# GuoleiSun/VSS-CFFM

Measured on AMD Instinct MI355X. Metric: clips/sec (fwd+bwd) CFFM-B1 480x480 T=4 hot path (CFFA+CFM, decoder_focal depth 2), higher is better.
Workload: dtype f32 in/out, f32 accumulate; MFMA operands: split-bf16 (hi+lo, ~2^-17) in the Linear GEMMs, f16 in QK^T/AV

## Files before the change

vss_cffm_amd/csrc/cffm_hip.hip:

```cpp
#include "cfm_attn_kernels.h"
#include "clip_kernels.h"
#include "rowops_kernels.h"
#include "gtc_kernels.h"
#include "gemm.h"
#include "segfuse_kernels.h"
#include "segloss_kernels.h"
#include "headfuse_kernels.h"

#include <stdarg.h>
#include <stdio.h>

#include "../../include/cffm_hip.h"

static thread_local char g_err[512] = "";

static int fail(int code, const char* fmt, ...) {
    va_list ap;
    va_start(ap, fmt);
    vsnprintf(g_err, sizeof(g_err), fmt, ap);
    va_end(ap);
    return code;
}
#define CHECK_LAUNCH(name)                                                                        \
    do {                                                                                          \
// ... 873 lines not shown
    ScratchFor pool(stream);
    PROF(ST_GEMM);
    if (gemm_tn_group((const GemmTN*)problems, n, (hipStream_t)stream)) return fail(-3, "linear_bwd_weight_group: gemm failed");
    CHECK_LAUNCH("linear_bwd_weight_group");
    return 0;
}

long cffm_tfrag_floats(long R, int C) { return R < 0 || C < 16 ? 0 : ((R + 31) / 32) * 32 * (long)C; }
int cffm_tfrag_pack(const float* x, float* dst, long R, int C, void* stream) {
    REQUIRE(x && dst && R >= 1 && C >= 16 && C % 16 == 0, "tfrag_pack: C must be a multiple of 16");
    const long items = ((R + 31) / 32) * (C / 16) * 64;
    CFFM_LAUNCH(k_tfrag_pack, ((unsigned)((items + 255) / 256)), (256), 0, (hipStream_t)stream, x, R, C, 0, (f32x4*)dst, items);
    CHECK_LAUNCH("tfrag_pack");
    return 0;
}
int cffm_linear_bwd_weight_tfrag_group(const cffm_wgrad* problems, int n, void* stream) {
    REQUIRE(problems && n >= 1 && n <= DWS_MAX, "linear_bwd_weight_tfrag_group: 1..%d problems", DWS_MAX);
    for (int i = 0; i < n; ++i) REQUIRE(problems[i].dy && problems[i].x && problems[i].dw, "linear_bwd_weight_tfrag_group: null operand");
    PROF(ST_GEMM);
    DwsPlan P;
    REQUIRE(dw_stream_plan((const GemmTN*)problems, n, dw_stream_target(), &P), "linear_bwd_weight_tfrag_group: N must be a multiple of 64, K of 128, operands under 4 GB");
    float* part = P.part_floats ? lib_scratch(P.part_floats) : nullptr;
    REQUIRE(!P.part_floats || part, "linear_bwd_weight_tfrag_group: scratch allocation failed");
    REQUIRE(!dw_group_stream((const GemmTN*)problems, n, (hipStream_t)stream, part, dw_stream_target()), "linear_bwd_weight_tfrag_group: launch failed");
    CHECK_LAUNCH("linear_bwd_weight_tfrag_group");
    return 0;
}
int cffm_linear_bwd_weight_tfrag(const float* dy_t, const float* x_t, float* dw, long M, int N, int K, void* stream) {
    const cffm_wgrad pr = {dy_t, x_t, dw, M, N, K};
    return cffm_linear_bwd_weight_tfrag_group(&pr, 1, stream);
}

int cffm_linear_qkv_fwd(const float* x, const float* w, const float* b, void* qkv16, long M, void* stream) {
    REQUIRE(x && w && b && qkv16, "linear_qkv_fwd: null");
    PROF(ST_GEMM);
    return gemm_nt_qkv16_split(x, w, b, (h16*)qkv16, M, 768, CFFM_C, (hipStream_t)stream) ? fail(-3, "linear_qkv_fwd: gemm failed") : 0;
}

int cffm_colsum(const float* a, long rows, int cols, float* out, void* stream) {
    ScratchFor pool(stream);
    PROF(ST_COLSUM);
    hipStream_t st = (hipStream_t)stream;
    REQUIRE(a && out && cols >= 4 && cols % 4 == 0, "colsum: cols must be a multiple of 4");
    const int slices = (int)((rows + COLSUM_ROWS - 1) / COLSUM_ROWS);
    float* part = red_scratch((size_t)slices * cols, st);
    REQUIRE(part, "colsum: scratch allocation failed");
    CFFM_LAUNCH(k_colsum_partial, (slices), (256), 0, st, a, rows, cols, part);
    RedSegs segs;
    segs.nseg = 0;
    seg_add(segs, 0, cols, out, 0);
    reduce_records(part, slices, cols, cols, segs, st);
    CHECK_LAUNCH("colsum");
    return 0;
}

static int cffm_ln_bwd_residual(const float* x1, const float* mean, const float* rstd, const float* gamma, const float* dz2,
                                const float* dres, float* dx1, float* dgamma, float* dbeta, long nrows, int zero_grads,
                                float* dres_colsum, float* dx1_colsum, void* stream) {
    PROF(ST_LN_BWD);
    hipStream_t st = (hipStream_t)stream;
    const int rpb = LNB_ROWS;
    const int nblk = (int)((nrows + rpb - 1) / rpb);
    float* part = red_scratch((size_t)nblk * 1024, st);
    REQUIRE(part, "ln_bwd_residual: scratch allocation failed");
    CFFM_LAUNCH(k_ln_bwd_residual, (nblk), (256), 0, st, x1, mean, rstd, gamma, dz2, dres, dx1, part, nrows, rpb);
    RedSegs segs;
    segs.nseg = 0;
    seg_add(segs, 0, CFFM_C, dgamma, !zero_grads);
    seg_add(segs, CFFM_C, CFFM_C, dbeta, !zero_grads);
    seg_add(segs, 2 * CFFM_C, CFFM_C, dres_colsum, 0);
    seg_add(segs, 3 * CFFM_C, CFFM_C, dx1_colsum, 0);
    reduce_records(part, nblk, 1024, 1024, segs, st);
    CHECK_LAUNCH("ln_bwd_residual");
    return 0;
}


int cffm_adamw_step_rows(const cffm_adamw_chunk2* chunks, int nchunks, const float* grad_base, float* state, const float* sched,
                         double* consts, int nrows, const int* active_rows, int* ticket, void* stream) {
    static_assert(sizeof(cffm_adamw_chunk2) == sizeof(AdamwChunk2), "chunk layout");
    if (nchunks <= 0) return 0;
    REQUIRE(chunks && state && sched && consts && nrows >= 1, "adamw_step_rows: null table or no rows");
    PROF(ST_ADAMW);
    if (ticket) {
        CFFM_LAUNCH(k_adamw_rows_tick, ((unsigned)nchunks), (256), 0, (hipStream_t)stream, (const AdamwChunk2*)chunks, grad_base, state, sched, consts,
                    nrows, active_rows, ticket);
    } else {
        CFFM_LAUNCH(k_adamw_tick_rows, ((unsigned)((nrows + 63) / 64)), (64), 0, (hipStream_t)stream, state, sched, consts, nrows, active_rows);
        CFFM_LAUNCH(k_adamw_rows, ((unsigned)nchunks), (256), 0, (hipStream_t)stream, (const AdamwChunk2*)chunks, grad_base, (const float*)state, consts);
    }
    CHECK_LAUNCH("adamw_rows");
    return 0;
}

#ifndef GTM_WGS_FWD
#define GTM_WGS_FWD 512
#endif
#ifndef GTM_WGS_DQ
#define GTM_WGS_DQ 512
#endif
#ifndef GTM_WGS_DKV
#define GTM_WGS_DKV 256
#endif
int cffm_gtc_attn_fwd(const float* q_raw, const float* q_b, const float* kv_raw, const float* kv_b, float* o, float* lse,
                      int B, int T, int K, void* stream) {
    PROF(ST_GTC_FWD);
    REQUIRE(K >= 1 && K <= 256, "gtc_attn_fwd: K=%d outside 1..256", K);
#ifndef CFFM_EMU
    static bool granted = false;
    if (!granted) {
        REQUIRE(hipFuncSetAttribute((const void*)k_gtc_attn_fwd, hipFuncAttributeMaxDynamicSharedMemorySize, gtf_lds(256)) == hipSuccess, "gtc_attn_fwd: LDS grant failed");
        granted = true;
    }
#endif
    if (K <= 128) {
        const int tiles = (T + 15) / 16;
        int tpw = (tiles * CFFM_HEADS * B + 4 * GTM_WGS_FWD - 1) / (4 * GTM_WGS_FWD);
        if (tpw < 1) tpw = 1;
        const unsigned gx = (unsigned)((tiles + 4 * tpw - 1) / (4 * tpw));
        const int U = (K + 31) / 32;
        hipStream_t st = (hipStream_t)stream;
        f32x4* fr = (f32x4*)lib_scratch((size_t)B * CFFM_HEADS * gtm_frag_units(U) * 256);
        REQUIRE(fr, "gtc_attn_fwd: scratch allocation failed");
#define GTM_FWD(U_)                                                                                                                          \
        do {                                                                                                                             \
            if (U_ > 1) CFFM_LAUNCH(k_gtc_pack_frags<U_>, (CFFM_HEADS, B, 2 * U_), (256), 0, st, kv_raw, kv_b, fr, K);                   \
            CFFM_LAUNCH(k_gtc_attn_fwd_mfma<U_>, (gx, CFFM_HEADS, B), (256), 0, st, q_raw, q_b, (const f32x4*)(U_ > 1 ? fr : nullptr), kv_raw, kv_b, o, lse, T, K, tpw);   \
        } while (0)
        if (U == 1) GTM_FWD(1); else if (U == 2) GTM_FWD(2); else if (U == 3) GTM_FWD(3); else GTM_FWD(4);
#undef GTM_FWD
        CHECK_LAUNCH("gtc_attn_fwd");
        return 0;
    }
    CFFM_LAUNCH(k_gtc_attn_fwd, ((T + GTC_TOK - 1) / GTC_TOK, CFFM_HEADS, B), (256), (size_t)gtf_lds(K), (hipStream_t)stream, q_raw, q_b, kv_raw, kv_b, o,
                lse, T, K);
    CHECK_LAUNCH("gtc_attn_fwd");
    return 0;
}

int cffm_gtc_attn_bwd(const float* q_raw, const float* q_b, const float* kv_raw, const float* kv_b, const float* o,
                      const float* dout, const float* lse, float* dq_raw, float* dkv, int B, int T, int K, void* stream) {
    PROF(ST_GTC_BWD);
    hipStream_t st = (hipStream_t)stream;
    REQUIRE(K >= 1 && K <= 256 && B >= 1 && T >= 1, "gtc_attn_bwd: K=%d outside 1..256", K);
    if (K <= 128) {
        const int tiles = (T + 15) / 16, pairs = (T + 31) / 32, U = (K + 31) / 32;
        int tpw = (tiles * CFFM_HEADS * B + 4 * GTM_WGS_DQ - 1) / (4 * GTM_WGS_DQ), ppw = (pairs * CFFM_HEADS * B + 4 * GTM_WGS_DKV - 1) / (4 * GTM_WGS_DKV);
        if (tpw < 1) tpw = 1;
        if (ppw < 1) ppw = 1;
        const unsigned g1 = (unsigned)((tiles + 4 * tpw - 1) / (4 * tpw)), g2 = (unsigned)((pairs + 4 * ppw - 1) / (4 * ppw));
        const size_t nD = ((size_t)B * T * CFFM_HEADS + 63) / 64 * 64;
        const size_t nrecf = ((size_t)B * CFFM_HEADS * g2 * K * 64 + 63) / 64 * 64;
        float* scr = lib_scratch(nD + nrecf + (size_t)B * CFFM_HEADS * gtm_frag_units(U) * 256);
        REQUIRE(scr, "gtc_attn_bwd: scratch allocation failed");
        float* Dbuf = scr;
        float* rec = scr + nD;
        f32x4* fr = (f32x4*)(scr + nD + nrecf);
#ifndef CFFM_EMU
        static bool granted_m = false;
        if (!granted_m) {
            REQUIRE(hipFuncSetAttribute((const void*)k_gtc_attn_bwd_dkv_mfma<3>, hipFuncAttributeMaxDynamicSharedMemorySize, gtm_bwd_lds(4)) == hipSuccess &&
                    hipFuncSetAttribute((const void*)k_gtc_attn_bwd_dkv_mfma<4>, hipFuncAttributeMaxDynamicSharedMemorySize, gtm_bwd_lds(4)) == hipSuccess, "gtc_attn_bwd: LDS grant failed");
            granted_m = true;
        }
#endif
#define GTM_BWD(U_)                                                                                                                                              \
        do {                                                                                                                                                 \
            const f32x4* fq = U_ > 1 ? (const f32x4*)fr : nullptr;                                \
            if (U_ > 1) CFFM_LAUNCH(k_gtc_pack_frags<U_>, (CFFM_HEADS, B, 2 * U_), (256), 0, st, kv_raw, kv_b, fr, K);                                       \
// ... 223 lines not shown
    }
    TRY(cffm_gtc_attn_fwd(ws + W.qraw, p->qkv_b, ws + W.kvraw, p->kv_b, ws + W.ao, ws + W.lse, B, T, K, stream));
    TRY(cffm_mlp_fwd_tfrag(ws + W.ao, x, 0, (int)nt, wf + 256 * 256, wf + 2 * 256 * 256, wf + 2 * 256 * 256 + CFFM_HID * 256, p->proj_b, p->fc1_b, p->fc2_b,
                           p->norm2_w, p->norm2_b, ws + W.x1, nullptr, ws + W.mean2, ws + W.rstd2, ws + W.hraw, nullptr, out, ws + W.ao_t, ws + W.z2,
                           ws + W.act, nt, stream));
    return 0;
}

int cffm_gtc_block_backward(const cffm_gtc_params* p, const cffm_gtc_grads* g, const float* x, const float* centers, const float* dout,
                            float* dx, float* dcenters, float* ws, int B, int T, int K, void* stream) {
    TRY(gtc_check(p, x, centers, dout, ws, B, T, K, "gtc_block_backward"));
    REQUIRE(g && dx && dcenters && g->norm1_w && g->norm1_b && g->qkv_w && g->qkv_b && g->kv_w && g->kv_b && g->proj_w && g->proj_b && g->norm2_w &&
            g->norm2_b && g->fc1_w && g->fc1_b && g->fc2_w && g->fc2_b, "gtc_block_backward: null gradient");
    hipStream_t st = (hipStream_t)stream;
    const long nt = (long)B * T, nk = (long)B * K;
    const GtcWs W = gtc_ws_layout(nt, nk);
    float* wn = ws + W.wn;
    TRY(gtc_pack(p, wn, 1, stream));
#ifdef CFFM_EMU
    memset(g->qkv_w + 256 * 256, 0, sizeof(float) * 512 * 256);
    memset(g->qkv_b + 256, 0, sizeof(float) * 512);
#else
    REQUIRE(hipMemsetAsync(g->qkv_w + 256 * 256, 0, sizeof(float) * 512 * 256, st) == hipSuccess &&
            hipMemsetAsync(g->qkv_b + 256, 0, sizeof(float) * 512, st) == hipSuccess, "gtc_block_backward: memset failed");
#endif
    RedScope reductions(st);
    TRY(cffm_mlp_bwd_tfrag(dout, ws + W.hraw, p->fc1_b, ws + W.x1, ws + W.mean2, ws + W.rstd2, p->norm2_w, wn + 2 * 256 * 256 + CFFM_HID * 256,
                           wn + 2 * 256 * 256, wn + 256 * 256, nullptr, ws + W.dx1, ws + W.dao, g->norm2_w, g->norm2_b, g->fc1_b, g->fc2_b, g->proj_b,
                           ws + W.dout_t, ws + W.dh, ws + W.dx1_t, nt, stream));
    TRY(cffm_gtc_attn_bwd(ws + W.qraw, p->qkv_b, ws + W.kvraw, p->kv_b, ws + W.ao, ws + W.dao, ws + W.lse, ws + W.dq, ws + W.dkv, B, T, K, stream));
    {
        PROF(ST_GEMM);
        const int mt = panel_mt(nt);
        const long nrec = (nt + 16 * mt - 1) / (16 * mt);
        float* qrec = red_scratch((size_t)nrec * 256, st);
        REQUIRE(qrec, "gtc_block_backward: scratch allocation failed");
        float* dq_t = ws + W.dq_t;
        const int rc = mt == 3 ? panel_gemm_launch<3, 2, false, 0>(ws + W.dq, 256, nt, 256, wn, ws + W.dz, 256, nullptr, nullptr, st, qrec, dq_t)
                               : panel_gemm_launch<2, 2, false, 0>(ws + W.dq, 256, nt, 256, wn, ws + W.dz, 256, nullptr, nullptr, st, qrec, dq_t);
        REQUIRE(!rc, "gtc_block_backward: q input-gradient gemm failed");
        RedSegs segs;
        segs.nseg = 0;
        seg_add(segs, 0, 256, g->qkv_b, 0);
        reduce_records(qrec, (int)nrec, 256, 256, segs, st);
    }
    {
        PROF(ST_GEMM); PROF2(ST_G_DW);
        const cffm_wgrad wt4[4] = {{ws + W.dq_t, ws + W.z_t, g->qkv_w, nt, 256, 256}, {ws + W.dh, ws + W.z2, g->fc1_w, nt, CFFM_HID, 256},
                                   {ws + W.dout_t, ws + W.act, g->fc2_w, nt, 256, CFFM_HID}, {ws + W.dx1_t, ws + W.ao_t, g->proj_w, nt, 256, 256}};
        DwsPlan P;
        REQUIRE(dw_stream_plan((const GemmTN*)wt4, 4, dw_stream_target(), &P), "gtc_block_backward: weight-gradient plan failed");
        float* part = P.part_floats ? lib_scratch(P.part_floats) : nullptr;
        REQUIRE(!P.part_floats || part, "gtc_block_backward: scratch allocation failed");
        REQUIRE(!dw_group_stream((const GemmTN*)wt4, 4, st, part, dw_stream_target()), "gtc_block_backward: weight-gradient gemm failed");
    }
    TRY(cffm_colsum(ws + W.dkv, nk, 512, g->kv_b, stream));
    {
        PROF(ST_GEMM);
        REQUIRE(!gemm_tn(ws + W.dkv, ws + W.cn, g->kv_w, nk, 512, 256, st), "gtc_block_backward: kv weight-gradient gemm failed");
        REQUIRE(!gemm_nn(ws + W.dkv, p->kv_w, ws + W.dcn, nk, 512, 256, st), "gtc_block_backward: kv input-gradient gemm failed");
    }
    TRY(cffm_ln_bwd_residual(x, ws + W.mean1, ws + W.rstd1, p->norm1_w, ws + W.dz, ws + W.dx1, dx, g->norm1_w, g->norm1_b, nt, 1, nullptr, nullptr, stream));
    reductions.finish();
    TRY(cffm_ln_bwd_residual(centers, ws + W.cmean, ws + W.crstd, p->norm1_w, ws + W.dcn, nullptr, dcenters, g->norm1_w, g->norm1_b, nk, 0, nullptr, nullptr,
                             stream));
    CHECK_LAUNCH("gtc_block_backward");
    return 0;
}

static int prep_args(PrepArgs& a, const cffm_block_params* params, int d0, int nd, float* ws0, long ws_stride, const cffm_block_ws& L) {
    const int nb = (CFFM_HEADS * CFFM_NQ_PAD * CFFM_NKEY_PAD + 255) / 256;
    for (int d = 0; d < PREP_MAXD; ++d) {
        const cffm_block_params& p = params[d0 + (d < nd ? d : 0)];
        float* ws = ws0 + (long)(d0 + (d < nd ? d : 0)) * ws_stride;
        a.t[d].own = p.rpb_own; a.t[d].ring = p.rpb_ring;
        for (int i = 0; i < 4; ++i) { a.t[d].pool[i] = p.rpb_pool[i]; a.pw[d].w[i] = p.pool_w[i]; }
        a.bias[d] = ws + L.bias; a.M[d] = ws + L.M;
        a.w[d][0] = p.qkv_w; a.w[d][1] = p.proj_w; a.w[d][2] = p.fc1_w; a.w[d][3] = p.fc2_w;
        a.w_s[d] = ws + L.w_split;
        a.w_f[d] = ws + L.w_frag;
    }
    a.nbias = nb;
    a.pack = 2;
    return nb + 1 + PREP_WBLOCKS + PREP_FBLOCKS;
}
static int param_prep(const cffm_block_params* params, int n, float* ws0, long ws_stride, const cffm_block_ws& L, void* stream) {
    PROF(ST_BIAS_ASM);
    for (int d0 = 0; d0 < n; d0 += PREP_MAXD) {
        const int nd = (n - d0 < PREP_MAXD) ? n - d0 : PREP_MAXD;
        PrepArgs a;
        const int pnx = prep_args(a, params, d0, nd, ws0, ws_stride, L);
        CFFM_LAUNCH(k_param_prep, (pnx, nd), (256), 0, (hipStream_t)stream, a);
    }
    CHECK_LAUNCH("param_prep");
    return 0;
}

static int block_forward_impl(const cffm_geom* g, const cffm_block_params* p, const float* x_ref, long ref_bs,
                              const float* x_tgt, long tgt_bs, const int* key_src, const int* q_dst, float* ws,
                              float* scratch, void* stream);
int cffm_block_forward(const cffm_geom* g, const cffm_block_params* p, const float* x_ref, long ref_bs,
                       const float* x_tgt, long tgt_bs, const int* key_src, const int* q_dst, float* ws,
                       float* scratch, void* stream) {
    REQUIRE(g && p && ws && scratch, "block_forward: null");
    cffm_block_ws L;
    cffm_block_ws_layout(g, &L);
    TRY(param_prep(p, 1, ws, 0, L, stream));
    return block_forward_impl(g, p, x_ref, ref_bs, x_tgt, tgt_bs, key_src, q_dst, ws, scratch, stream);
}
static struct { bool pending; hipStream_t side; } g_prep_join = {false, nullptr};
static int block_forward_impl(const cffm_geom* g, const cffm_block_params* p, const float* x_ref, long ref_bs,
                              const float* x_tgt, long tgt_bs, const int* key_src, const int* q_dst, float* ws,
                              float* scratch, void* stream) {
    cffm_block_ws L;
    cffm_block_ws_layout(g, &L);
    const long NR = (long)g->B * g->RC, NP = (long)g->B * g->HW;
    hipStream_t st = (hipStream_t)stream;
    const bool late_join = g_prep_join.pending;
    TRY(ln_pool_fwd_impl(g, x_ref, ref_bs, x_tgt, tgt_bs, p->norm1_w, p->norm1_b, ws + L.M, p->pool_b, ws + L.zall,
                         ws + L.mean1, ws + L.rstd1, 1, stream, late_join ? p->pool_w : nullptr));
    if (late_join) {
        g_prep_join.pending = false;
        side_join(g_prep_join.side, st, 0);
    }
    {
        PROF(ST_GEMM); PROF2(ST_G_QKV_FWD);
        REQUIRE(!panel_qkv_fwd(ws + L.zall, ws + L.w_frag, p->qkv_b, (h16*)(ws + L.qkv), NR, st, dw_stream_sw() ? ws + L.zall_t : nullptr), "block_forward: qkv gemm failed");
    }
    TRY(cffm_attn_fwd(g, ws + L.qkv, key_src, q_dst, (const void*)(ws + L.bias), ws + L.ao, ws + L.lse, stream));
    {
        const float* wf = ws + L.w_frag;
        PROF(ST_GEMM);
        if (dw_stream_sw())
            TRY(cffm_mlp_fwd_tfrag(ws + L.ao, x_tgt, tgt_bs, g->HW, wf + 768 * 256, wf + 768 * 256 + 256 * 256, wf + 768 * 256 + 256 * 256 + 1024 * 256,
                                   p->proj_b, p->fc1_b, p->fc2_b, p->norm2_w, p->norm2_b, ws + L.x1, nullptr, ws + L.mean2, ws + L.rstd2, ws + L.hraw,
                                   nullptr, ws + L.x2, ws + L.ao_t, ws + L.z2, ws + L.act, NP, stream));
        else
        TRY(cffm_mlp_fwd(ws + L.ao, x_tgt, tgt_bs, g->HW, wf + 768 * 256, wf + 768 * 256 + 256 * 256, wf + 768 * 256 + 256 * 256 + 1024 * 256,
                         p->proj_b, p->fc1_b, p->fc2_b, p->norm2_w, p->norm2_b, ws + L.x1, ws + L.z2, ws + L.mean2, ws + L.rstd2, ws + L.hraw,
                         ws + L.act, ws + L.x2, NP, stream));
        CHECK_LAUNCH("block_forward");
    }
    (void)scratch;
    return 0;
}

static int block_backward_impl(const cffm_geom* g, const cffm_block_params* p, const cffm_block_grads* gr,
                               const float* x_ref, long ref_bs, const float* x_tgt, long tgt_bs, const int* key_src,
                               const int* q_dst, const int* inv_ptr, const int* inv_idx, const float* ws, const float* dout,
                               float* dx_tgt, long dtgt_bs, float* scratch, int defer, int par, int slot, int nslots, void* stream);
#ifndef CFFM_EMU
static struct { bool has; RedJobs jobs; int parity; } g_tail = {false, {}, 0};
static int tail_flush(hipStream_t st) {
    if (!g_tail.has) return 0;
    g_tail.has = false;
    hipStream_t s3 = side_fork_take(st, 3);
    (void)hipStreamWaitEvent(s3, g_side.tail_order, 0);
    redq_launch(g_tail.jobs, s3);
    CHECK_LAUNCH("block_backward reductions");
    if (s3 != st) {
        side_record(s3, st, g_side.tail_done[g_tail.parity]);
        g_side.tail_pending[g_tail.parity] = true;
    }
    return 0;
}
#else
static int tail_flush(hipStream_t) { return 0; }
// ... 613 lines not shown
int cffm_vc_counts(const long long* gt, const long long* pred, int F, long npix, int n, long long* counts, void* stream) {
    REQUIRE(F >= 0 && npix >= 0 && n >= 1 && npix < (1L << 31), "vc_counts: bad sizes");
    if (F - n <= 0 || !npix) return 0;
    REQUIRE(gt && pred && counts, "vc_counts: null");
    REQUIRE(F - n <= 65535, "vc_counts: more than 65535 start frames in one call");
    CFFM_LAUNCH(k_vc_counts, ((unsigned)((npix + 255) / 256), (unsigned)(F - n)), (256), 0, (hipStream_t)stream, gt, pred, npix, n,
                (unsigned long long*)counts);
    CHECK_LAUNCH("vc_counts");
    return 0;
}

int cffm_layer_forward_rows(const cffm_geom* g, int depth, const cffm_block_params* params, const float* x_rows, float* y_rows,
                            const int* key_src, const int* q_dst, float* saved, float* scratch, void* stream) {
    REQUIRE(g && params && x_rows && y_rows && saved && scratch && depth >= 1, "layer_forward_rows: bad arguments");
    cffm_block_ws L;
    cffm_block_ws_layout(g, &L);
    const long HW = g->HW, img = HW * CFFM_C;
    float* blk0 = saved + up((long)g->B * 4 * img);
    TRY(param_prep(params, depth, blk0, L.total, L, stream));
    for (int i = 0; i < depth; ++i) {
        float* ws = blk0 + (long)i * L.total;
        const float* tgt = (i == 0) ? x_rows + 3 * img : blk0 + (long)(i - 1) * L.total + L.x2;
        const long tgt_bs = (i == 0) ? 4 * img : img;
        TRY(block_forward_impl(g, &params[i], x_rows, 4 * img, tgt, tgt_bs, key_src, q_dst, ws, scratch, stream));
    }
#ifdef CFFM_EMU
    memcpy(y_rows, blk0 + (long)(depth - 1) * L.total + L.x2, (size_t)g->B * img * sizeof(float));
#else
    REQUIRE(hipMemcpyAsync(y_rows, blk0 + (long)(depth - 1) * L.total + L.x2, (size_t)g->B * img * sizeof(float), hipMemcpyDeviceToDevice,
                           (hipStream_t)stream) == hipSuccess, "layer_forward_rows: copy failed");
#endif
    return 0;
}
int cffm_layer_backward_rows(const cffm_geom* g, int depth, const cffm_block_params* params, const cffm_block_grads* grads,
                             const float* x_rows, const float* dy_rows, float* dx_rows, const int* key_src, const int* q_dst,
                             const int* inv_ptr, const int* inv_idx, const float* saved, float* scratch, void* stream) {
    REQUIRE(g && params && grads && x_rows && dy_rows && dx_rows && saved && scratch && depth >= 1, "layer_backward_rows: bad arguments");
    cffm_block_ws L;
    cffm_block_ws_layout(g, &L);
    const Scratch S = scratch_layout(g);
    const long HW = g->HW, img = HW * CFFM_C;
    const float* blk0 = saved + up((long)g->B * 4 * img);
    tail_reset();
    for (int i = depth - 1; i >= 0; --i) {
        const float* ws = blk0 + (long)i * L.total;
        const float* tgt = (i == 0) ? x_rows + 3 * img : blk0 + (long)(i - 1) * L.total + L.x2;
        const long tgt_bs = (i == 0) ? 4 * img : img;
        float* dtgt = (i == 0) ? dx_rows + 3 * img : scratch + (((depth - i) & 1) ? S.a2 : S.a);
        const long dtgt_bs = (i == 0) ? 4 * img : img;
        const float* dout = (i == depth - 1) ? dy_rows : scratch + (((depth - 1 - i) & 1) ? S.a2 : S.a);
        TRY(block_backward_impl(g, &params[i], &grads[i], x_rows, 4 * img, tgt, tgt_bs, key_src, q_dst, inv_ptr, inv_idx, ws, dout, dtgt, dtgt_bs,
                                scratch, 1, (depth - 1 - i) & 1, i, depth, stream));
    }
    RedJobs* tail_jobs = nullptr;
#ifndef CFFM_EMU
    if (g_tail.has) {
        g_tail.has = false;
        tail_jobs = &g_tail.jobs;
    }
#endif
    TRY(cffa_finish(g, depth, params, grads, depth - 1, 0, blk0, L.total, x_rows, 4 * img, dx_rows, 4 * img, 0, stream, tail_jobs));
    side_join_all((hipStream_t)stream);
    return 0;
}

static int layer_forward_impl(const cffm_geom* g, int depth, const cffm_block_params* params, const float* x_nchw,
                              float* y_tgt_nchw, long y_bs, float* y_full, const int* key_src, const int* q_dst, float* saved,
                              float* scratch, void* stream) {
    REQUIRE(g && params && x_nchw && y_tgt_nchw && saved && scratch && depth >= 1, "layer_forward: bad arguments");
    cffm_block_ws L;
    cffm_block_ws_layout(g, &L);
    const long HW = g->HW, img = HW * CFFM_C;
    float* xs = saved;
    float* blk0 = saved + up((long)g->B * 4 * img);
    hipStream_t st = (hipStream_t)stream;
    side_init(st);
    if (depth <= PREP_MAXD) {
        PROF(ST_TRANSPOSE);
        PrepArgs a;
        const int pnx = prep_args(a, params, 0, depth, blk0, L.total, L);
        TrArgs T;
        T.src = x_nchw; T.dst = xs; T.rows = CFFM_C; T.cols = (int)HW; T.src_bs = img; T.dst_bs = img; T.add_mod = 4; T.add_skip = 3; T.copy_dst = y_full;
        T.gx = ((int)HW + 63) / 64; T.gy = (CFFM_C + 63) / 64; T.gz = g->B * 4;
        CFFM_LAUNCH(k_transpose_prep, ((unsigned)(T.gx * T.gy * T.gz + pnx * depth)), (256), 0, st, T, a, pnx);
        CHECK_LAUNCH("transpose + param_prep");
        g_prep_join.pending = false;
    } else {
        side_fork_mark(st, 0);
        TRY(transpose_add(x_nchw, xs, g->B * 4, CFFM_C, (int)HW, img, img, nullptr, 4, 3, stream, y_full));
        hipStream_t sd = side_fork_take(st, 0);
        TRY(param_prep(params, depth, blk0, L.total, L, (void*)sd));
        side_mark(sd, st, 0);
        g_prep_join.pending = sd != st;
        g_prep_join.side = sd;
    }
#ifndef CFFM_EMU
    g_side.used = 0;
#endif
    for (int i = 0; i < depth; ++i) {
        float* ws = blk0 + (long)i * L.total;
        const float* tgt = (i == 0) ? xs + 3 * img : blk0 + (long)(i - 1) * L.total + L.x2;
        const long tgt_bs = (i == 0) ? 4 * img : img;
        TRY(block_forward_impl(g, &params[i], xs, 4 * img, tgt, tgt_bs, key_src, q_dst, ws, scratch, stream));
    }
    TRY(cffm_transpose(blk0 + (long)(depth - 1) * L.total + L.x2, y_tgt_nchw, g->B, (int)HW, CFFM_C, img, y_bs, stream));
    return 0;
}
int cffm_layer_forward(const cffm_geom* g, int depth, const cffm_block_params* params, const float* x_nchw,
                       float* y_tgt_nchw, const int* key_src, const int* q_dst, float* saved, float* scratch,
                       void* stream) {
    REQUIRE(g, "layer_forward: bad arguments");
    return layer_forward_impl(g, depth, params, x_nchw, y_tgt_nchw, g->HW * CFFM_C, nullptr, key_src, q_dst, saved, scratch, stream);
}
int cffm_layer_forward_full(const cffm_geom* g, int depth, const cffm_block_params* params, const float* x_nchw,
                            float* y_full_nchw, const int* key_src, const int* q_dst, float* saved, float* scratch,
                            void* stream) {
    REQUIRE(g && y_full_nchw && y_full_nchw != x_nchw, "layer_forward_full: bad arguments");
    const long img = g->HW * CFFM_C;
    return layer_forward_impl(g, depth, params, x_nchw, y_full_nchw + 3 * img, 4 * img, y_full_nchw, key_src, q_dst, saved, scratch, stream);
}

static int layer_backward_impl(const cffm_geom* g, int depth, const cffm_block_params* params, const cffm_block_grads* grads,
                               const float* dy_tgt_nchw, long dy_bs, const float* dy_full, float* dx_nchw, const int* key_src,
                               const int* q_dst, const int* inv_ptr, const int* inv_idx, const float* saved, float* scratch,
                               int first_block, int last_block, void* stream) {
    REQUIRE(g && params && grads && dy_tgt_nchw && dx_nchw && saved && scratch && depth >= 1, "layer_backward: bad arguments");
    REQUIRE(first_block < depth && last_block >= 0 && first_block >= last_block, "layer_backward: bad block range %d..%d of %d", first_block,
            last_block, depth);
    cffm_block_ws L;
    cffm_block_ws_layout(g, &L);
    const Scratch S = scratch_layout(g);
    const long HW = g->HW, img = HW * CFFM_C;
    const float* xs = saved;
    const float* blk0 = saved + up((long)g->B * 4 * img);
    float* dxs = scratch + S.dxs;
    REQUIRE(dy_bs >= img, "layer_backward: dy batch stride %ld < %ld", dy_bs, img);
    if (first_block == depth - 1) TRY(cffm_transpose(dy_tgt_nchw, scratch + S.a, g->B, CFFM_C, (int)HW, dy_bs, img, stream));
    tail_reset();
    for (int i = first_block; i >= last_block; --i) {
        const float* ws = blk0 + (long)i * L.total;
        const float* tgt = (i == 0) ? xs + 3 * img : blk0 + (long)(i - 1) * L.total + L.x2;
        const long tgt_bs = (i == 0) ? 4 * img : img;
        float* dcur = scratch + (((depth - 1 - i) & 1) ? S.a2 : S.a);
        float* dtgt = (i == 0) ? dxs + 3 * img : scratch + (((depth - i) & 1) ? S.a2 : S.a);
        const long dtgt_bs = (i == 0) ? 4 * img : img;
        TRY(block_backward_impl(g, &params[i], &grads[i], xs, 4 * img, tgt, tgt_bs, key_src, q_dst, inv_ptr, inv_idx, ws, dcur, dtgt, dtgt_bs, scratch,
                                1, (depth - 1 - i) & 1, i, depth, stream));
    }
    RedJobs* tail_jobs = nullptr;
#ifndef CFFM_EMU
    if (last_block == 0 && g_tail.has) {
        g_tail.has = false;
        tail_jobs = &g_tail.jobs;
    }
#endif
    TRY(cffa_finish(g, depth, params, grads, first_block, last_block, blk0, L.total, xs, 4 * img, dxs, 4 * img, first_block != depth - 1, stream, tail_jobs));
    if (last_block == 0) TRY(transpose_add(dxs, dx_nchw, g->B * 4, (int)HW, CFFM_C, img, img, dy_full, 4, 3, stream));
    TRY(tail_flush((hipStream_t)stream));
    side_join_all((hipStream_t)stream);
    return 0;
}
int cffm_layer_backward_range(const cffm_geom* g, int depth, const cffm_block_params* params, const cffm_block_grads* grads,
                              const float* dy_tgt_nchw, long dy_bs, float* dx_nchw, const int* key_src, const int* q_dst,
                              const int* inv_ptr, const int* inv_idx, const float* saved, float* scratch, int first_block,
                              int last_block, void* stream) {
    return layer_backward_impl(g, depth, params, grads, dy_tgt_nchw, dy_bs, nullptr, dx_nchw, key_src, q_dst, inv_ptr, inv_idx, saved,
                               scratch, first_block, last_block, stream);
// ... 22 lines not shown
```

vss_cffm_amd/csrc/rowops_kernels.h:

```cpp
#pragma once
#include "cffm_common.h"
#include "cffa_kernels.h"
#include "panel_kernels.h"

struct BiasTables {
    const float* own;
    const float* ring;
    const float* pool[4];
};
struct BiasTablesG {
    float* own;
    float* ring;
    float* pool[4];
};

__device__ __forceinline__ int bias_locate(int h, int q, int n, int& off) {
    const int qi = q / 7, qj = q % 7;
    if (n < 49) {
        const int ki = n / 7, kj = n % 7;
        off = ((qi - ki + 6) * 13 + (qj - kj + 6)) * CFFM_HEADS + h;
        return 0;
    }
    if (n < 181) {
        off = (h * 49 + q) * 132 + (n - 49);
        return 1;
    }
    int base, kk, id;
    if (n < 206) { base = 181; kk = 5; id = 2; }
    else if (n < 255) { base = 206; kk = 7; id = 3; }
    else if (n < 280) { base = 255; kk = 5; id = 4; }
    else { base = 280; kk = 3; id = 5; }
    const int a = (n - base) / kk, bb = (n - base) % kk, side = 6 + kk;
    off = h * side * side + (qi - a + kk - 1) * side + (qj - bb + kk - 1);
    return id;
}

__device__ __forceinline__ long biash_index(int h, int q, int n) {
    const int t = n >> 4;
    return ((long)((h * 4 + (q >> 4)) * 10 + (t >> 1)) * 64 + (((t & 1) * 2 + ((n >> 3) & 1)) * 16 + (q & 15))) * 8 + (n & 7);
}
__device__ __forceinline__ void bias_assemble_body(const BiasTables& t, float* __restrict__ bias, h16* __restrict__ biasH, int bx) {
    const int e = bx * 256 + threadIdx.x;
    if (e >= CFFM_HEADS * CFFM_NQ_PAD * CFFM_NKEY_PAD) return;
    const int n = e % CFFM_NKEY_PAD, q = (e / CFFM_NKEY_PAD) % CFFM_NQ_PAD, h = e / (CFFM_NKEY_PAD * CFFM_NQ_PAD);
    float v = 0.f;
    if (q < CFFM_WA && n < CFFM_NKEY) {
        int off;
        const int id = bias_locate(h, q, n, off);
        v = id == 0 ? t.own[off] : id == 1 ? t.ring[off] : t.pool[id - 2][off];
    }
    if (bias) bias[e] = v;
    if (biasH) {
        biasH[biash_index(h, q, n)] = (h16)v;
        if (n >= CFFM_NKEY_PAD - 16) biasH[biash_index(h, q, n + 16)] = (h16)0.f;
    }
}
__global__ void __launch_bounds__(256) k_bias_assemble(BiasTables t, float* __restrict__ bias, h16* __restrict__ biasH) {
    bias_assemble_body(t, bias, biasH, blockIdx.x);
}
#define PREP_MAXD 4
#define PREP_WFLOATS (768 * 256 + 256 * 256 + 1024 * 256 + 256 * 1024)
#define PREP_WBLOCKS (PREP_WFLOATS / 4 / 256)
#define PREP_FBLOCKS (2 * PREP_WFLOATS / 8 / 256)
struct PrepArgs {
    BiasTables t[PREP_MAXD];
    PoolW pw[PREP_MAXD];
    float* bias[PREP_MAXD];
    float* M[PREP_MAXD];
    const float* w[PREP_MAXD][4];
    float* w_s[PREP_MAXD];
    float* w_f[PREP_MAXD];
    int nbias, pack;
};
__device__ __forceinline__ void param_prep_body(const PrepArgs& a, int bx, int d) {
    if (bx < a.nbias) { bias_assemble_body(a.t[d], nullptr, (h16*)a.bias[d], bx); return; }
    if (bx == a.nbias) { pool_matrix_body(a.pw[d], a.M[d]); return; }
    if (!a.pack) return;
    const long n4[4] = {768 * 256 / 4, 256 * 256 / 4, 1024 * 256 / 4, 256 * 1024 / 4};
    if (bx >= a.nbias + 1 + PREP_WBLOCKS) {
        long it = (long)(bx - a.nbias - 1 - PREP_WBLOCKS) * 256 + threadIdx.x;
        const int form = it >= PREP_WFLOATS / 8;
        if (form) it -= PREP_WFLOATS / 8;
        const int N[4] = {768, 256, 1024, 256}, K[4] = {256, 256, 256, 1024};
        long o8 = 0;
#pragma unroll
        for (int k = 0; k < 4; ++k) {
            if (it >= o8 && it < o8 + n4[k] / 2)
                pnl_pack_weight(a.w[d][k], N[k], K[k], form != 0, (f32x4*)(a.w_f[d] + (long)form * PREP_WFLOATS + o8 * 8), it - o8);
            o8 += n4[k] / 2;
        }
        return;
    }
    if (a.pack == 2) return;
    long e = (long)(bx - a.nbias - 1) * 256 + threadIdx.x;
    long off = 0;
#pragma unroll
    for (int k = 0; k < 4; ++k) {
        if (e >= off && e < off + n4[k]) ((f32x4*)a.w_s[d])[e] = split4_pack(((const f32x4*)a.w[d][k])[e - off]);
        off += n4[k];
    }
}
__global__ void __launch_bounds__(256) k_param_prep(PrepArgs a) { param_prep_body(a, blockIdx.x, blockIdx.y); }
struct TrArgs { const float* src; float* dst; int rows, cols; long src_bs, dst_bs; int add_mod, add_skip; float* copy_dst; int gx, gy, gz; };
__global__ void __launch_bounds__(256) k_transpose_prep(TrArgs T, PrepArgs a, int pnx) {
    const int nt = T.gx * T.gy * T.gz;
    int b = blockIdx.x;
    if (b < nt) {
        transpose_body(T.src, T.dst, T.rows, T.cols, T.src_bs, T.dst_bs, nullptr, T.add_mod, T.add_skip, T.copy_dst, b % T.gx, (b / T.gx) % T.gy,
                       b / (T.gx * T.gy));
        return;
    }
    b -= nt;
    param_prep_body(a, b % pnx, b / pnx);
}

__global__ void __launch_bounds__(256) k_bias_scatter(const float* __restrict__ dbiasT, BiasTablesG g) {
    const int e = blockIdx.x * 256 + threadIdx.x;
    const int n_own = 169 * CFFM_HEADS, n_ring = CFFM_HEADS * 49 * 132;
    if (e < n_ring) {
        const int n = e % 132, q = (e / 132) % 49, h = e / (132 * 49);
        g.ring[e] = dbiasT[((long)h * CFFM_NKEY_PAD + 49 + n) * CFFM_NQ_PAD + q];
    }
    if (blockIdx.x * 256 + 255 < n_ring) return;
    const int j = (e - n_ring) & 15;
    int r = (e - n_ring) >> 4;
    float acc = 0.f;
    float* dst = nullptr;
    if (e < n_ring) {
        r = -1;
    } else if (r < n_own) {
        const int h = r % CFFM_HEADS, idx = r / CFFM_HEADS, di = idx / 13 - 6, dj = idx % 13 - 6;
#pragma unroll
        for (int u = 0; u < 4; ++u) {
            const int q = j + 16 * u, ki = q / 7 - di, kj = q % 7 - dj;
            if (q < 49 && ki >= 0 && ki < 7 && kj >= 0 && kj < 7) acc += dbiasT[((long)h * CFFM_NKEY_PAD + ki * 7 + kj) * CFFM_NQ_PAD + q];
        }
        dst = g.own + r;
    } else {
        r -= n_own;
        const int kks[4] = {5, 7, 5, 3}, bases[4] = {181, 206, 255, 280};
#pragma unroll
        for (int t = 0; t < 4; ++t) {
            const int kk = kks[t], side = 6 + kk, n_t = CFFM_HEADS * side * side;
            if (!dst && r >= 0 && r < n_t) {
                const int h = r / (side * side), idx = r % (side * side), di = idx / side - (kk - 1), dj = idx % side - (kk - 1);
#pragma unroll
                for (int u = 0; u < 4; ++u) {
                    const int q = j + 16 * u, a = q / 7 - di, bb = q % 7 - dj;
                    if (q < 49 && a >= 0 && a < kk && bb >= 0 && bb < kk)
                        acc += dbiasT[((long)h * CFFM_NKEY_PAD + bases[t] + a * kk + bb) * CFFM_NQ_PAD + q];
                }
                dst = g.pool[t] + r;
            }
            r -= n_t;
        }
    }
    acc = row16_sum(acc);
    if (dst && j == 0) *dst = acc;
}
#define BIAS_SCATTER_THREADS (CFFM_HEADS * 49 * 132 + 16 * (169 * CFFM_HEADS + CFFM_HEADS * (121 + 169 + 121 + 81)))

#define LNB_ROWS 16
__global__ void __launch_bounds__(256) k_ln_bwd_residual(const float* __restrict__ x1, const float* __restrict__ mean_in,
                                                          const float* __restrict__ rstd_in, const float* __restrict__ gamma,
                                                          const float* __restrict__ dz2, const float* __restrict__ dres,
                                                          float* __restrict__ dx1, float* __restrict__ part, long nrows,
                                                          int rows_per_block) {
    __shared__ float red[4][4][CFFM_C];
    const int lane = threadIdx.x & 63, wave = threadIdx.x >> 6;
    const f32x4 gm = *(const f32x4*)(gamma + 4 * lane);
    const f32x4 z4 = (f32x4){0.f, 0.f, 0.f, 0.f};
    f32x4 ag = z4, ab = z4, ar = z4, ax = z4;
    const long r0 = (long)blockIdx.x * LNB_ROWS;
    constexpr int RW = LNB_ROWS / 4;
    f32x4 xr[RW], dzr[RW], drr[RW];
    float mur[RW], rsr[RW];
#pragma unroll
    for (int k = 0; k < RW; ++k) {
        const long row = r0 + wave + 4 * k;
        xr[k] = dzr[k] = drr[k] = z4;
        mur[k] = rsr[k] = 0.f;
        if (row < nrows) {
            xr[k] = *(const f32x4*)(x1 + row * CFFM_C + 4 * lane);
            dzr[k] = *(const f32x4*)(dz2 + row * CFFM_C + 4 * lane);
            if (dres) drr[k] = *(const f32x4*)(dres + row * CFFM_C + 4 * lane);
            mur[k] = mean_in[row];
            rsr[k] = rstd_in[row];
        }
    }
#pragma unroll
    for (int k = 0; k < RW; ++k) {
        const long row = r0 + wave + 4 * k;
        if (row >= nrows) break;
        const float rs = rsr[k];
        const f32x4 xh = (xr[k] - mur[k]) * rs;
        const f32x4 dz = dzr[k];
// ... 140 lines not shown
    if (s < nsplit) a += ((const f32x4*)(part + (long)s * n))[i];
    ((f32x4*)G.out[p])[i] = a + b;
}


#define ADAMW_NCONST 12
struct AdamwChunk2 { float* p; const float* g; float* m; float* v; int n; int row; };
__device__ __forceinline__ double adamw_ipow(double b, double t) {
    long n = (long)t;
    double r = 1.0;
    while (n > 0) {
        if (n & 1) r *= b;
        b *= b;
        n >>= 1;
    }
    return r;
}
__device__ __forceinline__ void adamw_next_state(const float* __restrict__ state, const float* __restrict__ sched, const double* __restrict__ consts,
                                                 int r, float out[4]) {
    const double* c = consts + (long)ADAMW_NCONST * r;
    const double t = (double)state[4 * r] + 1.0, wd = (double)sched[2 * r + 1];
    double lr = (double)sched[2 * r];
    if (c[3] == 1.0) {
        const double it = c[10] - c[9], max_iters = c[4], min_lr = c[6], wi = c[7];
        const double frac = it < max_iters ? 1.0 - it / max_iters : 0.0;
        lr = (lr - min_lr) * (c[5] == 1.0 ? frac : pow(frac, c[5])) + min_lr;
        if (it < wi) lr *= 1.0 - (1.0 - it / wi) * (1.0 - c[8]);
        if (it < 0.0) lr = 0.0;
    }
    out[0] = (float)t;
    out[1] = (float)(lr / (1.0 - adamw_ipow(c[0], t)));
    out[2] = (float)(1.0 / sqrt(1.0 - adamw_ipow(c[1], t)));
    out[3] = (float)(1.0 - lr * wd);
}
__global__ void k_adamw_tick_rows(float* __restrict__ state, const float* __restrict__ sched, double* __restrict__ consts, int nrows,
                                  const int* __restrict__ active) {
    const int r = blockIdx.x * blockDim.x + threadIdx.x;
    if (r >= nrows) return;
    if (!active || active[r]) {
        float o[4];
        adamw_next_state(state, sched, consts, r, o);
        state[4 * r] = o[0]; state[4 * r + 1] = o[1]; state[4 * r + 2] = o[2]; state[4 * r + 3] = o[3];
    }
    consts[ADAMW_NCONST * r + 10] += 1.0;
}
__device__ __forceinline__ void adamw_elem(float& p, float& m, float& v, float g, float beta1, float omb1, float beta2, float omb2, float decay,
                                           float step_size, float inv_sqrt_bc2, float eps) {
#ifdef __clang__
#pragma clang fp contract(off)
#endif
    m = beta1 * m + omb1 * g;
    v = beta2 * v + omb2 * g * g;
    p = p * decay - step_size * (m / (sqrtf(v) * inv_sqrt_bc2 + eps));
}
__device__ __forceinline__ void adamw_update_chunk(AdamwChunk2 c, const float* __restrict__ grad_base, float step_size, float inv_sqrt_bc2,
                                                   float decay, const double* __restrict__ consts) {
    if (grad_base) c.g = (const float*)((const char*)grad_base + (uintptr_t)c.g);
    const double b1 = consts[ADAMW_NCONST * c.row], b2 = consts[ADAMW_NCONST * c.row + 1];
    const float beta1 = (float)b1, beta2 = (float)b2, omb1 = (float)(1.0 - b1), omb2 = (float)(1.0 - b2), eps = (float)consts[ADAMW_NCONST * c.row + 2];
    const bool vec = (((uintptr_t)c.p | (uintptr_t)c.g | (uintptr_t)c.m | (uintptr_t)c.v) & 15) == 0;
    const int n4 = vec ? c.n / 4 : 0;
    for (int e = threadIdx.x; e < n4; e += 256) {
        f32x4 p = ((const f32x4*)c.p)[e], m = ((const f32x4*)c.m)[e], v = ((const f32x4*)c.v)[e];
        const f32x4 g = ((const f32x4*)c.g)[e];
#pragma unroll
        for (int k = 0; k < 4; ++k) {
            float pk = p[k], mk = m[k], vk = v[k];
            adamw_elem(pk, mk, vk, g[k], beta1, omb1, beta2, omb2, decay, step_size, inv_sqrt_bc2, eps);
            p[k] = pk; m[k] = mk; v[k] = vk;
        }
        ((f32x4*)c.p)[e] = p; ((f32x4*)c.m)[e] = m; ((f32x4*)c.v)[e] = v;
    }
    for (int e = 4 * n4 + threadIdx.x; e < c.n; e += 256) {
        float pk = c.p[e], mk = c.m[e], vk = c.v[e];
        adamw_elem(pk, mk, vk, c.g[e], beta1, omb1, beta2, omb2, decay, step_size, inv_sqrt_bc2, eps);
        c.m[e] = mk; c.v[e] = vk; c.p[e] = pk;
    }
}
__global__ void __launch_bounds__(256) k_adamw_rows(const AdamwChunk2* __restrict__ chunks, const float* __restrict__ grad_base,
                                                     const float* __restrict__ state, const double* __restrict__ consts) {
    const AdamwChunk2 c = chunks[blockIdx.x];
    adamw_update_chunk(c, grad_base, state[4 * c.row + 1], state[4 * c.row + 2], state[4 * c.row + 3], consts);
}
__global__ void __launch_bounds__(256) k_adamw_rows_tick(const AdamwChunk2* __restrict__ chunks, const float* __restrict__ grad_base,
                                                          float* __restrict__ state, const float* __restrict__ sched,
                                                          double* __restrict__ consts, int nrows, const int* __restrict__ active,
                                                          int* __restrict__ ticket) {
    __shared__ float sc[4];
    __shared__ int last;
    AdamwChunk2 c = chunks[blockIdx.x];
    const bool full = c.n == 2048 && (((uintptr_t)c.p | (uintptr_t)(grad_base ? (const float*)((const char*)grad_base + (uintptr_t)c.g) : c.g) | (uintptr_t)c.m | (uintptr_t)c.v) & 15) == 0;
    if (full) {
        if (grad_base) c.g = (const float*)((const char*)grad_base + (uintptr_t)c.g);
        const int e0 = threadIdx.x, e1 = threadIdx.x + 256;
        f32x4 p0 = ((const f32x4*)c.p)[e0], m0 = ((const f32x4*)c.m)[e0], v0 = ((const f32x4*)c.v)[e0], p1 = ((const f32x4*)c.p)[e1],
              m1 = ((const f32x4*)c.m)[e1], v1 = ((const f32x4*)c.v)[e1];
        const f32x4 g0 = ((const f32x4*)c.g)[e0], g1 = ((const f32x4*)c.g)[e1];
        if (threadIdx.x == 0) adamw_next_state(state, sched, consts, c.row, sc);
        __syncthreads();
        const float step_size = sc[1], inv_sqrt_bc2 = sc[2], decay = sc[3];
        const double b1 = consts[ADAMW_NCONST * c.row], b2 = consts[ADAMW_NCONST * c.row + 1];
        const float beta1 = (float)b1, beta2 = (float)b2, omb1 = (float)(1.0 - b1), omb2 = (float)(1.0 - b2), eps = (float)consts[ADAMW_NCONST * c.row + 2];
#pragma unroll
        for (int k = 0; k < 4; ++k) {
            float pk = p0[k], mk = m0[k], vk = v0[k];
            adamw_elem(pk, mk, vk, g0[k], beta1, omb1, beta2, omb2, decay, step_size, inv_sqrt_bc2, eps);
            p0[k] = pk; m0[k] = mk; v0[k] = vk;
            pk = p1[k]; mk = m1[k]; vk = v1[k];
            adamw_elem(pk, mk, vk, g1[k], beta1, omb1, beta2, omb2, decay, step_size, inv_sqrt_bc2, eps);
            p1[k] = pk; m1[k] = mk; v1[k] = vk;
        }
        ((f32x4*)c.p)[e0] = p0; ((f32x4*)c.m)[e0] = m0; ((f32x4*)c.v)[e0] = v0;
        ((f32x4*)c.p)[e1] = p1; ((f32x4*)c.m)[e1] = m1; ((f32x4*)c.v)[e1] = v1;
    } else {
        if (threadIdx.x == 0) adamw_next_state(state, sched, consts, c.row, sc);
        __syncthreads();
        adamw_update_chunk(c, grad_base, sc[1], sc[2], sc[3], consts);
    }
    if (threadIdx.x == 0) {
        const int slot = blockIdx.x & 63, quota = ((int)gridDim.x - slot + 63) / 64, nslots = (int)gridDim.x < 64 ? (int)gridDim.x : 64;
        int l = 0;
        if (atomicAdd(ticket + 1 + slot, 1) == quota - 1) {
            ticket[1 + slot] = 0;
            l = atomicAdd(ticket, 1) == nslots - 1;
        }
        last = l;
    }
    __syncthreads();
    if (!last) return;
    for (int r = threadIdx.x; r < nrows; r += 256) {
        if (!active || active[r]) {
            float o[4];
            adamw_next_state(state, sched, consts, r, o);
            state[4 * r] = o[0]; state[4 * r + 1] = o[1]; state[4 * r + 2] = o[2]; state[4 * r + 3] = o[3];
        }
        consts[ADAMW_NCONST * r + 10] += 1.0;
    }
    if (threadIdx.x == 0) *ticket = 0;
}
```

Before: 2933.

## Persistent AdamW with LDS row-state table and prefetch; reorder param prep blocks

The AdamW tick kernel becomes persistent. It uses a capped grid, and each workgroup first computes per-row schedule state for all rows into LDS, then loops over chunks with a grid stride, prefetching the next chunk's p/m/v/g registers while updating the current one. The last workgroup writes back the cached row state instead of recomputing it. Separately, the pool-matrix prep becomes per-element blocks scheduled first in the fused transpose+prep launch, and the block count is computed by a helper. Every workgroup now redundantly computes state for all rows, and register pressure rises from double-buffered chunk data.

```diff
diff --git a/vss_cffm_amd/csrc/cffm_hip.hip b/vss_cffm_amd/csrc/cffm_hip.hip
--- a/vss_cffm_amd/csrc/cffm_hip.hip
+++ b/vss_cffm_amd/csrc/cffm_hip.hip
@@ -979,9 +979,11 @@
     if (nchunks <= 0) return 0;
     REQUIRE(chunks && state && sched && consts && nrows >= 1, "adamw_step_rows: null table or no rows");
     PROF(ST_ADAMW);
-    if (ticket) {
-        CFFM_LAUNCH(k_adamw_rows_tick, ((unsigned)nchunks), (256), 0, (hipStream_t)stream, (const AdamwChunk2*)chunks, grad_base, state, sched, consts,
-                    nrows, active_rows, ticket);
+    if (ticket && nrows <= ADAMW_LDS_ROWS) {
+        int wgs = (nchunks + ADAMW_CHUNKS_PER_WG - 1) / ADAMW_CHUNKS_PER_WG;
+        if (wgs > ADAMW_MAX_WGS) wgs = ADAMW_MAX_WGS;
+        CFFM_LAUNCH(k_adamw_rows_tick, ((unsigned)wgs), (256), 0, (hipStream_t)stream, (const AdamwChunk2*)chunks, nchunks, grad_base, state, sched,
+                    consts, nrows, active_rows, ticket);
     } else {
         CFFM_LAUNCH(k_adamw_tick_rows, ((unsigned)((nrows + 63) / 64)), (64), 0, (hipStream_t)stream, state, sched, consts, nrows, active_rows);
         CFFM_LAUNCH(k_adamw_rows, ((unsigned)nchunks), (256), 0, (hipStream_t)stream, (const AdamwChunk2*)chunks, grad_base, (const float*)state, consts);
@@ -1371,7 +1373,7 @@
     }
     a.nbias = nb;
     a.pack = 2;
-    return nb + 1 + PREP_WBLOCKS + PREP_FBLOCKS;
+    return prep_blocks(nb, a.pack);
 }
 static int param_prep(const cffm_block_params* params, int n, float* ws0, long ws_stride, const cffm_block_ws& L, void* stream) {
     PROF(ST_BIAS_ASM);
@@ -2151,7 +2153,7 @@
         TrArgs T;
         T.src = x_nchw; T.dst = xs; T.rows = CFFM_C; T.cols = (int)HW; T.src_bs = img; T.dst_bs = img; T.add_mod = 4; T.add_skip = 3; T.copy_dst = y_full;
         T.gx = ((int)HW + 63) / 64; T.gy = (CFFM_C + 63) / 64; T.gz = g->B * 4;
-        CFFM_LAUNCH(k_transpose_prep, ((unsigned)(T.gx * T.gy * T.gz + pnx * depth)), (256), 0, st, T, a, pnx);
+        CFFM_LAUNCH(k_transpose_prep, ((unsigned)(T.gx * T.gy * T.gz + pnx * depth)), (256), 0, st, T, a, pnx, depth);
         CHECK_LAUNCH("transpose + param_prep");
         g_prep_join.pending = false;
     } else {
diff --git a/vss_cffm_amd/csrc/rowops_kernels.h b/vss_cffm_amd/csrc/rowops_kernels.h
--- a/vss_cffm_amd/csrc/rowops_kernels.h
+++ b/vss_cffm_amd/csrc/rowops_kernels.h
@@ -72,13 +72,20 @@
     float* w_f[PREP_MAXD];
     int nbias, pack;
 };
+#define PREP_PBLOCKS ((CFFM_NCELL * CFFM_WA + 255) / 256)
+__host__ __device__ __forceinline__ int prep_blocks(int nbias, int pack) {
+    return PREP_PBLOCKS + (pack ? PREP_FBLOCKS : 0) + (pack == 1 ? PREP_WBLOCKS : 0) + nbias;
+}
 __device__ __forceinline__ void param_prep_body(const PrepArgs& a, int bx, int d) {
-    if (bx < a.nbias) { bias_assemble_body(a.t[d], nullptr, (h16*)a.bias[d], bx); return; }
-    if (bx == a.nbias) { pool_matrix_body(a.pw[d], a.M[d]); return; }
-    if (!a.pack) return;
+    if (bx < PREP_PBLOCKS) {
+        const int e = bx * 256 + threadIdx.x;
+        if (e < CFFM_NCELL * CFFM_WA) a.M[d][e] = pool_matrix_entry(a.pw[d], e / CFFM_WA, e % CFFM_WA);
+        return;
+    }
+    bx -= PREP_PBLOCKS;
     const long n4[4] = {768 * 256 / 4, 256 * 256 / 4, 1024 * 256 / 4, 256 * 1024 / 4};
-    if (bx >= a.nbias + 1 + PREP_WBLOCKS) {
-        long it = (long)(bx - a.nbias - 1 - PREP_WBLOCKS) * 256 + threadIdx.x;
+    if (a.pack && bx < PREP_FBLOCKS) {
+        long it = (long)bx * 256 + threadIdx.x;
         const int form = it >= PREP_WFLOATS / 8;
         if (form) it -= PREP_WFLOATS / 8;
         const int N[4] = {768, 256, 1024, 256}, K[4] = {256, 256, 256, 1024};
@@ -91,27 +98,40 @@
         }
         return;
     }
-    if (a.pack == 2) return;
-    long e = (long)(bx - a.nbias - 1) * 256 + threadIdx.x;
-    long off = 0;
-#pragma unroll
-    for (int k = 0; k < 4; ++k) {
-        if (e >= off && e < off + n4[k]) ((f32x4*)a.w_s[d])[e] = split4_pack(((const f32x4*)a.w[d][k])[e - off]);
-        off += n4[k];
-    }
+    if (a.pack) bx -= PREP_FBLOCKS;
+    if (a.pack == 1) {
+        if (bx < PREP_WBLOCKS) {
+            const long e = (long)bx * 256 + threadIdx.x;
+            long off = 0;
+#pragma unroll
+            for (int k = 0; k < 4; ++k) {
+                if (e >= off && e < off + n4[k]) ((f32x4*)a.w_s[d])[e] = split4_pack(((const f32x4*)a.w[d][k])[e - off]);
+                off += n4[k];
+            }
+            return;
+        }
+        bx -= PREP_WBLOCKS;
+    }
+    if (bx < a.nbias) bias_assemble_body(a.t[d], nullptr, (h16*)a.bias[d], bx);
 }
 __global__ void __launch_bounds__(256) k_param_prep(PrepArgs a) { param_prep_body(a, blockIdx.x, blockIdx.y); }
 struct TrArgs { const float* src; float* dst; int rows, cols; long src_bs, dst_bs; int add_mod, add_skip; float* copy_dst; int gx, gy, gz; };
-__global__ void __launch_bounds__(256) k_transpose_prep(TrArgs T, PrepArgs a, int pnx) {
+__global__ void __launch_bounds__(256) k_transpose_prep(TrArgs T, PrepArgs a, int pnx, int nd) {
     const int nt = T.gx * T.gy * T.gz;
     int b = blockIdx.x;
+    if (b < PREP_PBLOCKS * nd) {
+        param_prep_body(a, b % PREP_PBLOCKS, b / PREP_PBLOCKS);
+        return;
+    }
+    b -= PREP_PBLOCKS * nd;
     if (b < nt) {
         transpose_body(T.src, T.dst, T.rows, T.cols, T.src_bs, T.dst_bs, nullptr, T.add_mod, T.add_skip, T.copy_dst, b % T.gx, (b / T.gx) % T.gy,
                        b / (T.gx * T.gy));
         return;
     }
     b -= nt;
-    param_prep_body(a, b % pnx, b / pnx);
+    const int rest = pnx - PREP_PBLOCKS;
+    param_prep_body(a, PREP_PBLOCKS + b % rest, b / rest);
 }
 
 __global__ void __launch_bounds__(256) k_bias_scatter(const float* __restrict__ dbiasT, BiasTablesG g) {
@@ -418,40 +438,70 @@
     const AdamwChunk2 c = chunks[blockIdx.x];
     adamw_update_chunk(c, grad_base, state[4 * c.row + 1], state[4 * c.row + 2], state[4 * c.row + 3], consts);
 }
-__global__ void __launch_bounds__(256) k_adamw_rows_tick(const AdamwChunk2* __restrict__ chunks, const float* __restrict__ grad_base,
+#define ADAMW_LDS_ROWS 256
+#define ADAMW_CHUNKS_PER_WG 2
+#define ADAMW_MAX_WGS 1024
+struct AdamwFull { f32x4 p[2], m[2], v[2], g[2]; };
+__device__ __forceinline__ bool adamw_full(AdamwChunk2& c, const float* __restrict__ grad_base) {
+    if (grad_base) c.g = (const float*)((const char*)grad_base + (uintptr_t)c.g);
+    return c.n == 2048 && (((uintptr_t)c.p | (uintptr_t)c.g | (uintptr_t)c.m | (uintptr_t)c.v) & 15) == 0;
+}
+__device__ __forceinline__ void adamw_load_full(const AdamwChunk2& c, AdamwFull& r) {
+#pragma unroll
+    for (int h = 0; h < 2; ++h) {
+        const int e = threadIdx.x + 256 * h;
+        r.p[h] = ((const f32x4*)c.p)[e]; r.m[h] = ((const f32x4*)c.m)[e]; r.v[h] = ((const f32x4*)c.v)[e]; r.g[h] = ((const f32x4*)c.g)[e];
+    }
+}
+__global__ void __launch_bounds__(256) k_adamw_rows_tick(const AdamwChunk2* __restrict__ chunks, int nchunks, const float* __restrict__ grad_base,
                                                           float* __restrict__ state, const float* __restrict__ sched,
                                                           double* __restrict__ consts, int nrows, const int* __restrict__ active,
                                                           int* __restrict__ ticket) {
-    __shared__ float sc[4];
+    __shared__ float sc[ADAMW_LDS_ROWS][8];
+    __shared__ float seps[ADAMW_LDS_ROWS];
     __shared__ int last;
-    AdamwChunk2 c = chunks[blockIdx.x];
-    const bool full = c.n == 2048 && (((uintptr_t)c.p | (uintptr_t)(grad_base ? (const float*)((const char*)grad_base + (uintptr_t)c.g) : c.g) | (uintptr_t)c.m | (uintptr_t)c.v) & 15) == 0;
-    if (full) {
-        if (grad_base) c.g = (const float*)((const char*)grad_base + (uintptr_t)c.g);
-        const int e0 = threadIdx.x, e1 = threadIdx.x + 256;
-        f32x4 p0 = ((const f32x4*)c.p)[e0], m0 = ((const f32x4*)c.m)[e0], v0 = ((const f32x4*)c.v)[e0], p1 = ((const f32x4*)c.p)[e1],
-              m1 = ((const f32x4*)c.m)[e1], v1 = ((const f32x4*)c.v)[e1];
-        const f32x4 g0 = ((const f32x4*)c.g)[e0], g1 = ((const f32x4*)c.g)[e1];
-        if (threadIdx.x == 0) adamw_next_state(state, sched, consts, c.row, sc);
-        __syncthreads();
-        const float step_size = sc[1], inv_sqrt_bc2 = sc[2], decay = sc[3];
-        const double b1 = consts[ADAMW_NCONST * c.row], b2 = consts[ADAMW_NCONST * c.row + 1];
-        const float beta1 = (float)b1, beta2 = (float)b2, omb1 = (float)(1.0 - b1), omb2 = (float)(1.0 - b2), eps = (float)consts[ADAMW_NCONST * c.row + 2];
-#pragma unroll
-        for (int k = 0; k < 4; ++k) {
-            float pk = p0[k], mk = m0[k], vk = v0[k];
-            adamw_elem(pk, mk, vk, g0[k], beta1, omb1, beta2, omb2, decay, step_size, inv_sqrt_bc2, eps);
-            p0[k] = pk; m0[k] = mk; v0[k] = vk;
-            pk = p1[k]; mk = m1[k]; vk = v1[k];
-            adamw_elem(pk, mk, vk, g1[k], beta1, omb1, beta2, omb2, decay, step_size, inv_sqrt_bc2, eps);
-            p1[k] = pk; m1[k] = mk; v1[k] = vk;
-        }
-        ((f32x4*)c.p)[e0] = p0; ((f32x4*)c.m)[e0] = m0; ((f32x4*)c.v)[e0] = v0;
-        ((f32x4*)c.p)[e1] = p1; ((f32x4*)c.m)[e1] = m1; ((f32x4*)c.v)[e1] = v1;
-    } else {
-        if (threadIdx.x == 0) adamw_next_state(state, sched, consts, c.row, sc);
-        __syncthreads();
-        adamw_update_chunk(c, grad_base, sc[1], sc[2], sc[3], consts);
+    int ci = blockIdx.x;
+    AdamwChunk2 c = chunks[ci];
+    bool full = adamw_full(c, grad_base);
+    AdamwFull cur;
+    if (full) adamw_load_full(c, cur);
+    for (int r = threadIdx.x; r < nrows; r += 256) {
+        float o[4];
+        adamw_next_state(state, sched, consts, r, o);
+        const double b1 = consts[ADAMW_NCONST * r], b2 = consts[ADAMW_NCONST * r + 1];
+        sc[r][0] = o[0]; sc[r][1] = o[1]; sc[r][2] = o[2]; sc[r][3] = o[3];
+        sc[r][4] = (float)b1; sc[r][5] = (float)(1.0 - b1); sc[r][6] = (float)b2; sc[r][7] = (float)(1.0 - b2);
+        seps[r] = (float)consts[ADAMW_NCONST * r + 2];
+    }
+    __syncthreads();
+    while (ci < nchunks) {
+        const int nci = ci + (int)gridDim.x;
+        AdamwChunk2 nc = c;
+        bool nfull = false;
+        AdamwFull nxt;
+        if (nci < nchunks) {
+            nc = chunks[nci];
+            nfull = adamw_full(nc, grad_base);
+            if (nfull) adamw_load_full(nc, nxt);
+        }
+        const float* f = sc[c.row];
+        const float step_size = f[1], inv_sqrt_bc2 = f[2], decay = f[3], beta1 = f[4], omb1 = f[5], beta2 = f[6], omb2 = f[7], eps = seps[c.row];
+        if (full) {
+#pragma unroll
+            for (int h = 0; h < 2; ++h) {
+#pragma unroll
+                for (int k = 0; k < 4; ++k) {
+                    float pk = cur.p[h][k], mk = cur.m[h][k], vk = cur.v[h][k];
+                    adamw_elem(pk, mk, vk, cur.g[h][k], beta1, omb1, beta2, omb2, decay, step_size, inv_sqrt_bc2, eps);
+                    cur.p[h][k] = pk; cur.m[h][k] = mk; cur.v[h][k] = vk;
+                }
+                const int e = threadIdx.x + 256 * h;
+                ((f32x4*)c.p)[e] = cur.p[h]; ((f32x4*)c.m)[e] = cur.m[h]; ((f32x4*)c.v)[e] = cur.v[h];
+            }
+        } else {
+            adamw_update_chunk(c, nullptr, step_size, inv_sqrt_bc2, decay, consts);
+        }
+        ci = nci; c = nc; full = nfull; cur = nxt;
     }
     if (threadIdx.x == 0) {
         const int slot = blockIdx.x & 63, quota = ((int)gridDim.x - slot + 63) / 64, nslots = (int)gridDim.x < 64 ? (int)gridDim.x : 64;
@@ -466,9 +516,7 @@
     if (!last) return;
     for (int r = threadIdx.x; r < nrows; r += 256) {
         if (!active || active[r]) {
-            float o[4];
-            adamw_next_state(state, sched, consts, r, o);
-            state[4 * r] = o[0]; state[4 * r + 1] = o[1]; state[4 * r + 2] = o[2]; state[4 * r + 3] = o[3];
+            state[4 * r] = sc[r][0]; state[4 * r + 1] = sc[r][1]; state[4 * r + 2] = sc[r][2]; state[4 * r + 3] = sc[r][3];
         }
         consts[ADAMW_NCONST * r + 10] += 1.0;
     }
```

Result: no change. 2954 (median of 6 runs) (+0.7%).
